# drnatebrown/col-bwt

Measured on AMD Instinct MI355X. Metric: query bases/s, higher is better.
Workload: dtype int64

## Files before the change

### col-bwt_amd/__init__.py

```python
import ctypes as C
import os

import numpy as np

_HERE = os.path.dirname(os.path.abspath(__file__))
LIB_PATH = os.path.join(_HERE, "libcolbwt.so")
HEADER_PATH = os.path.join(os.path.dirname(_HERE), "include", "colbwt.h")

EXPORTS = (
    "colbwt_version", "colbwt_last_error", "colbwt_index_open", "colbwt_index_open_memory",
    "colbwt_index_open_layout", "colbwt_index_open_memory_layout",
    "colbwt_index_open_devices", "colbwt_index_open_memory_devices",
    "colbwt_index_close", "colbwt_index_info", "colbwt_query_batch", "colbwt_query_batch_u32",
    "colbwt_query_device", "colbwt_query_device_ordered", "colbwt_query_file", "colbwt_query_file_binary",
    "colbwt_binary_to_text", "colbwt_synth_index_bytes", "colbwt_synth_index", "colbwt_synth_index_thr", "colbwt_pml_pack_device", "colbwt_read_end_mask_device", "colbwt_pml_unpack_device",
    "colbwt_index_cid_dictionary", "colbwt_cid_code_bits", "colbwt_cid_pack_device", "colbwt_cid_unpack_device",
    "colbwt_synth_reads_device", "colbwt_build_col_pml", "colbwt_build_col_pml_arrays",
    "colbwt_col_split", "colbwt_col_split_arrays", "colbwt_col_split_error",
    "colbwt_rlbwt_build_text", "colbwt_rlbwt_build_files", "colbwt_rlbwt_get", "colbwt_rlbwt_free", "colbwt_rlbwt_error",
    "colbwt_count_batch", "colbwt_count_device", "colbwt_count_file",
    "colbwt_index_attach_locate", "colbwt_index_attach_locate_memory", "colbwt_locate_docs", "colbwt_locate_batch",
    "colbwt_locate_device", "colbwt_locate_file",
    "colbwt_rlbwt_build_text_locate", "colbwt_rlbwt_build_files_locate", "colbwt_rlbwt_write_locate",
)

LOCATE_NONE = (1 << 64) - 1


class ColbwtError(RuntimeError):
    def __init__(self, code, msg):
        super().__init__(f"colbwt error {code}: {msg}")
        self.code = code


class Info(C.Structure):
    _fields_ = [("bwt_r", C.c_uint64), ("n", C.c_uint64), ("r", C.c_uint64), ("sigma", C.c_uint32),
                ("device", C.c_uint32), ("device_bytes", C.c_uint64), ("layout", C.c_uint32),
                ("layout_shape", C.c_uint32), ("table_rows", C.c_uint64), ("n_devices", C.c_uint32),
                ("reserved_", C.c_uint32)]


class Stats(C.Structure):
    _fields_ = [("n_reads", C.c_uint64), ("n_bases", C.c_uint64), ("h2d_ms", C.c_double),
                ("kernel_ms", C.c_double), ("d2h_ms", C.c_double), ("algorithmic_bytes", C.c_uint64)]

    def as_dict(self):
        return {k: getattr(self, k) for k, _ in self._fields_}


_lib = None


def lib():
    global _lib
    if _lib is not None:
        return _lib
    if not os.path.exists(LIB_PATH):
        raise ColbwtError(-100, f"{LIB_PATH} not built: run __graft_entry__.build() "
                                "(the query path has no CPU fallback)")
    try:
        import torch
    except ImportError:
        pass
    L = C.CDLL(LIB_PATH)
    vp, u64, i32 = C.c_void_p, C.c_uint64, C.c_int
    L.colbwt_version.restype = C.c_char_p
    L.colbwt_last_error.restype = C.c_char_p
    L.colbwt_index_open.argtypes = [C.c_char_p, vp, i32, C.POINTER(vp)]
    L.colbwt_index_open_memory.argtypes = [vp, u64, vp, i32, C.POINTER(vp)]
    L.colbwt_index_open_layout.argtypes = [C.c_char_p, vp, i32, i32, C.POINTER(vp)]
    L.colbwt_index_open_memory_layout.argtypes = [vp, u64, vp, i32, i32, C.POINTER(vp)]
    L.colbwt_index_open_devices.argtypes = [C.c_char_p, vp, C.POINTER(i32), i32, i32, C.POINTER(vp)]
# ... 396 lines not shown
```

### col-bwt_amd/csrc/capi.hip

```cpp
#include <fcntl.h>
#include <hip/hip_runtime.h>
#include <stdlib.h>
#include <string.h>
#include <sys/mman.h>
#include <sys/stat.h>
#include <unistd.h>

#include <algorithm>
#include <atomic>
#include <chrono>
#include <condition_variable>
#include <deque>
#include <mutex>
#include <string>
#include <thread>
#include <vector>

#include "../../include/colbwt.h"
#include "bin_writer.h"
#include "count_query.h"
#include "fasta_parallel.h"
#include "fastx_reader.h"
#include "index.h"
#include "locate_query.h"
// ... 797 lines not shown
            const std::string msg = "replica on device " + std::to_string(devices[k]) + ": " + g_err;
            delete first;
            return fail(rc, msg);
        }
        first->more.push_back(rep);
    }
    *out = first;
    return COLBWT_OK;
}

int colbwt_index_open_devices(const char *prefix_or_file, const colbwt_widths *widths, const int *devices, int n_devices,
                              int layout, colbwt_index **out) {
    if (!prefix_or_file || !out) return fail(COLBWT_ERR_ARG, "null argument");
    *out = nullptr;
    MappedFile mf;
    const int rc = map_index_file(prefix_or_file, mf);
    return rc != COLBWT_OK ? rc : colbwt_index_open_memory_devices(mf.data, mf.len, widths, devices, n_devices, layout, out);
}

void colbwt_index_close(colbwt_index *idx) { delete idx; }

int colbwt_index_info(const colbwt_index *idx, colbwt_info *out) {
    if (!idx || !out) return fail(COLBWT_ERR_ARG, "null argument");
    out->bwt_r = idx->ix.bwt_r();
    out->n = idx->ix.n();
    out->r = idx->ix.r();
    out->sigma = idx->ix.sigma();
    out->device = (uint32_t)idx->ix.device();
    out->device_bytes = idx->ix.device_bytes() + idx->loc.bytes();
    out->layout = (uint32_t)idx->ix.layout();
    out->layout_shape = idx->ix.line_rows() ? (idx->ix.table_fat().steps << 8) | kFatSlotSteps : 0;
    out->table_rows = idx->ix.table_rows();
    out->n_devices = 1 + (uint32_t)idx->more.size();
    out->reserved_ = 0;
    return COLBWT_OK;
}

int colbwt_query_batch(colbwt_index *idx, const uint8_t *bases, const uint64_t *read_off, uint64_t n_reads,
                       uint16_t *pml, uint8_t *cid, colbwt_stats *stats) {
    return query_batch_all<uint16_t>(idx, bases, read_off, n_reads, pml, cid, stats);
}

int colbwt_query_batch_u32(colbwt_index *idx, const uint8_t *bases, const uint64_t *read_off, uint64_t n_reads,
                           uint32_t *pml, uint8_t *cid, colbwt_stats *stats) {
    return query_batch_all<uint32_t>(idx, bases, read_off, n_reads, pml, cid, stats);
}

int colbwt_query_device(colbwt_index *idx, const uint8_t *d_bases, const uint64_t *d_read_off, uint64_t n_reads,
                        uint64_t n_bases, void *d_pml, int pml_bytes, uint8_t *d_cid, void *hip_stream,
                        colbwt_stats *stats) {
    return colbwt_query_device_ordered(idx, d_bases, d_read_off, n_reads, n_bases, d_pml, pml_bytes, d_cid, nullptr,
                                       hip_stream, stats);
}

int colbwt_query_device_ordered(colbwt_index *idx, const uint8_t *d_bases, const uint64_t *d_read_off,
                                uint64_t n_reads, uint64_t n_bases, void *d_pml, int pml_bytes, uint8_t *d_cid,
                                const uint32_t *d_order, void *hip_stream, colbwt_stats *stats) {
    auto bad_argument = [&]() -> const char * {
        if (pml_bytes != 2 && pml_bytes != 4) return "pml_bytes must be 2 or 4";
        if (n_reads == 0) return nullptr;
        if (!d_bases || !d_read_off || !d_pml || !d_cid) return "null device pointer";
        if (((uintptr_t)d_bases & 15) || ((uintptr_t)d_pml & 31) || ((uintptr_t)d_cid & 15))
            return "d_bases/d_cid must be 16-byte aligned and d_pml 32-byte aligned";
        return nullptr;
    };
    return device_entry(idx, d_bases, n_reads, n_bases, hip_stream, kAlgBytesPerBase, stats, bad_argument,
                        [&](const Index &ix, hipStream_t stream) {
// ... 405 lines not shown
```

### col-bwt_amd/csrc/fat2_query.hip

```cpp
#include <hip/hip_runtime.h>
#include <stdint.h>

#include "device_layout.h"
#include "fat_cursor.h"
#include "fat_layout.h"
#include "lane_io.h"
#include "lane_out.h"
#include "query_kernels.h"

namespace colbwt {

namespace {

constexpr uint32_t kOffMis0 = 0xFFFFFFFCu;
constexpr uint32_t kOffMis1 = 0xFFFFFFFBu;

#ifdef COLBWT_COUNT_TRIPS
#define FAT2_STAT(k) (++stat[k])
#else
#define FAT2_STAT(k) ((void)0)
#endif

__device__ __forceinline__ uint32_t mis_slot(const uint8_t *top, uint32_t own, uint32_t c) {
    const uint32_t aidx = top[own], cidx = top[c];
    const uint32_t slot = cidx < aidx ? cidx : cidx - 1;
    return cidx < 4 && slot < kFatSlots ? slot : kFatSlots;
}

template <int K, typename PmlT, bool kDeep>
__global__ __launch_bounds__(kQueryBlock)
void fat2_query_kernel(FatTable T, const uint8_t *__restrict__ bases, const uint64_t *__restrict__ read_off,
                       uint64_t n_reads, uint32_t big_reads, uint32_t tail_permille,
                       PmlT *__restrict__ pml, uint8_t *__restrict__ cid) {
    constexpr bool kWide = sizeof(PmlT) == 4;
    __shared__ uint4 s_stage[kWaves][8][64];
    __shared__ uint4 s_win[kWaves][4][64];
    __shared__ uint32_t s_claim;
    __shared__ uint8_t s_top[256];
    const uint32_t wave = threadIdx.x >> 6, lane = threadIdx.x & 63u, g8 = lane & ~7u, p = lane & 7u;
    uint32_t *const s_jx = reinterpret_cast<uint32_t *>(&s_stage[wave][7][48]);
    ChunkPlan plan;
    plan.init(n_reads, big_reads, tail_permille);
    if (threadIdx.x == 0) s_claim = 0;
    s_top[threadIdx.x] = (uint8_t)fat_top_index(T.top4, threadIdx.x);
    __syncthreads();
    uint32_t *const claim = &s_claim;
    ReadCursor rc;
    bool done;
    rc.c_next = threadIdx.x;
    rc.request_chunk(plan, read_off);
    rc.commit();
    done = !rc.enter_chunk(plan, claim);

    OutRuns acc;
    uint32_t trip = 0;
    LaneWindow win;
    win.init(rc.off + rc.k - 1);
    uint4 (*const my_win)[64] = s_win[wave];

    uint32_t j = done ? 0u : T.r - 1;
    uint32_t o = kOffLastPos;
    uint32_t L = 0;
    const uint4 *const my_row = &s_stage[wave][p][g8];

#ifdef COLBWT_COUNT_TRIPS
    unsigned long long stat[8] = {0, 0, 0, 0, 0, 0, 0, 0};
#endif
    while (__any(!done)) {
        bool step_back = false;
        if (!done && rc.k == 0 && !rc.next_in_flight && (rc.r != rc.r_lo || rc.nc_ready)) {
            if (rc.r != rc.r_lo) {
                rc.r -= 1;
                rc.k = rc.off - rc.next_off;
                rc.off = rc.next_off;
                step_back = rc.r > rc.r_lo;
            } else if (kWide || acc.cnt == 0) {
                done = !rc.enter_chunk(plan, claim);
                if (!done) win.init(rc.off + rc.k - 1);
            }
            j = done ? 0u : T.r - 1;
            o = kOffLastPos;
            L = 0;
        }
        const bool live = !done && rc.k != 0;
        uint64_t &k = rc.k;
        const uint64_t g = rc.off + k - 1;

        s_jx[lane] = j;
        wave_sync();
        {
            const uint4 ja = *reinterpret_cast<const uint4 *>(&s_jx[g8]);
            const uint4 jb = *reinterpret_cast<const uint4 *>(&s_jx[g8 + 4]);
            const uint32_t jq[8] = {ja.x, ja.y, ja.z, ja.w, jb.x, jb.y, jb.z, jb.w};
            wave_sync();
#pragma unroll
            for (uint32_t q = 0; q < 8; ++q)
                __builtin_amdgcn_global_load_lds(T.lines + (uint64_t)jq[q] * kFatRowBytes + ((p ^ q) << 4), &s_stage[wave][q][0],
                                                 16, 0, 0);
        }
        if (live && win.avail(g) < (k < 8u ? (uint32_t)k : 8u)) win.request(my_win, bases, g);
        if (step_back) { rc.in_next = read_off[rc.r - 1]; rc.next_in_flight = true; }
        if (!done && rc.fetch_pending) rc.request_chunk(plan, read_off);
        lds_dma_landed();
        rc.commit();

        const uint32_t have = live ? win.avail(g) : 0u;
        uint32_t consumed = 0, l_new = 0, keep = 0xFFFFFFFFu, keep1 = 0xFFFFFFFFu;
        uint64_t ids = 0;
        if (!live || have == 0) FAT2_STAT(5);
        if (live && have != 0) {
            const uint64_t W = win.get8(my_win, lane, g);
            const uint32_t left = k < have ? (uint32_t)k : have;
            if (o == kOffMis0 || o == kOffMis1) {
                FAT2_STAT(2);
                const uint32_t h4 = !kDeep && o == kOffMis1 ? 4u : 0u;
                const uint4 e0 = my_row[(h4 + 0u) ^ p], e1 = my_row[(h4 + 1u) ^ p], e2 = my_row[(h4 + 2u) ^ p],
                            e3 = my_row[(h4 + 3u) ^ p];
                const uint32_t carry = L;
                const uint32_t t1 = (e0.y >> 16) & 0xFFu, d1 = e0.y >> 24, v1 = e3.z & 7u;
                uint32_t oc = 4;
                if (left >= 2) {
                    const uint32_t c2 = (uint32_t)(W >> 48) & 0xFFu;
                    const uint32_t s2 = mis_slot(s_top, t1, c2);
                    if (c2 == t1) oc = 0;
                    else if (s2 < kFatSlots && ((v1 >> s2) & 1u)) oc = 1 + s2;
                }
                if (oc < 4) {
                    const uint32_t J = oc == 0 ? e0.z : oc == 1 ? e0.w : oc == 2 ? e1.x : e1.y;
                    const uint32_t rho = oc == 0 ? e1.z : oc == 1 ? e1.w : oc == 2 ? e2.x : e2.y;
                    const uint32_t pw = oc < 2 ? e2.z : e2.w, P = (oc & 1u) ? pw >> 16 : pw & 0xFFFFu;
                    const uint32_t ch = (e3.x >> (8 * oc)) & 0xFFu, cd = (e3.y >> (8 * oc)) & 0xFFu;
                    const uint32_t vo = (e3.z >> (4 + 4 * oc)) & 7u;
                    consumed = 2;
                    l_new = 1;
                    keep = oc == 0 ? 0xFFFFFFFFu : 0u;
                    ids = (uint64_t)(d1 | (carry << 8));
                    L = oc == 0 ? 1u : 0u;
                    uint32_t nJ = J, nP = P, nrho = rho, nch = ch, ncd = cd, nv = vo, seen = 2;
                    if constexpr (kDeep) {
                        if (left >= 3 && ((uint32_t)(W >> 40) & 0xFFu) == ch) {
                            const uint4 f0 = my_row[4u ^ p], f1 = my_row[5u ^ p], f2 = my_row[6u ^ p], f3 = my_row[7u ^ p];
                            nJ = oc == 0 ? f0.x : oc == 1 ? f0.y : oc == 2 ? f0.z : f0.w;
                            nrho = oc == 0 ? f1.x : oc == 1 ? f1.y : oc == 2 ? f1.z : f1.w;
                            const uint32_t pw2 = oc < 2 ? f2.x : f2.y;
                            nP = (oc & 1u) ? pw2 >> 16 : pw2 & 0xFFFFu;
                            nch = (f2.z >> (8 * oc)) & 0xFFu;
// ... 90 lines not shown
                    } else {
                        consumed = steps - skip;
                        l_new = L + consumed;
                    }
                    L = l_new;
                    ids = steps ? CID >> (8u * (8u - steps)) : 0ull;
                    if (k == consumed) {
                    } else if (to_entry) {
                        FAT2_STAT(6);
                        j = T.slot_line0 + (kDeep ? e_next : e_next >> 1);
                        o = kDeep ? kOffMis0 : kOffMis0 - (e_next & 1u);
                        L = carry;
                    } else if (own_jump) {
                        const uint32_t e = steps - 1;
                        const uint32_t I = reinterpret_cast<const uint32_t *>(&my_row[((kFatI / 16) + (e >> 2)) ^ p])[e & 3u];
                        const uint32_t Oh = reinterpret_cast<const uint16_t *>(&my_row[((kFatO / 16) + (e >> 3)) ^ p])[e & 7u];
                        const uint64_t cuts = (uint64_t)r1.y | ((uint64_t)r1.z << 32);
                        const uint32_t cut = (uint32_t)(cuts >> (8 * e)) & 0xFFu, cut_a = cut & 0xFu, len_b = cut >> 4;
                        j = I;
                        if (cut_a != kSKCutNone && o >= cut_a) {
                            j += 1;
                            o -= cut_a;
                            if (len_b != kSKCutNone && o >= len_b) {
                                j += 1;
                                o -= len_b;
                            }
                        } else {
                            o += Oh;
                        }
                    }
                }
            }
            if constexpr (kWide) {
                for (uint32_t e = 0; e < consumed; ++e) {
                    pml[g - consumed + 1 + e] = (PmlT)((e < 2 ? keep : keep1) ? l_new - e : 0u);
                    cid[g - consumed + 1 + e] = (uint8_t)(ids >> (8 * e));
                }
            } else {
                acc.push_run(consumed, l_new, keep, keep1, (uint32_t)ids, (uint32_t)(ids >> 32));
            }
            k -= consumed;
        }
        wave_sync();
        if constexpr (!kWide) {
#ifdef COLBWT_ABL_NO_FLUSH
            if ((trip & (OutRuns::kPeriod - 1)) == OutRuns::kPeriod - 1) acc.cnt = acc.cnt > 90 ? 1 : 0;
#else
            if ((trip & (OutRuns::kPeriod - 1)) == OutRuns::kPeriod - 1)
                acc.flush_wave((uint16_t *)pml, cid, rc.off + rc.k, !done, rc.k == 0 && rc.r == rc.r_lo, &s_stage[wave][0][0], lane);
#endif
        }
        ++trip;
        wave_sync();
    }
#ifdef COLBWT_COUNT_TRIPS
    for (int q = 0; q < 8; ++q) atomicAdd(&g_fat_stats[q], stat[q]);
#endif
}

template <int K>
void launch_steps2(const FatTable &T, const uint8_t *d_bases, const uint64_t *d_read_off, uint64_t n_reads, uint64_t n_bases,
                   void *d_pml, int pml_bytes, uint8_t *d_cid, hipStream_t stream) {
    const bool deep = T.entry_shift == 7;
    if (pml_bytes == 2 && deep) launch_persistent<fat2_query_kernel<K, uint16_t, true>>(T, d_bases, d_read_off, n_reads, n_bases, (uint16_t *)d_pml, d_cid, stream);
    else if (pml_bytes == 2) launch_persistent<fat2_query_kernel<K, uint16_t, false>>(T, d_bases, d_read_off, n_reads, n_bases, (uint16_t *)d_pml, d_cid, stream);
    else if (deep) launch_persistent<fat2_query_kernel<K, uint32_t, true>>(T, d_bases, d_read_off, n_reads, n_bases, (uint32_t *)d_pml, d_cid, stream);
    else launch_persistent<fat2_query_kernel<K, uint32_t, false>>(T, d_bases, d_read_off, n_reads, n_bases, (uint32_t *)d_pml, d_cid, stream);
}

}

void launch_fat2_query(const FatTable &T, const uint8_t *d_bases, const uint64_t *d_read_off, uint64_t n_reads, uint64_t n_bases,
// ... 21 lines not shown
```

### col-bwt_amd/csrc/fat_build.hip

```cpp
#include <hip/hip_runtime.h>
#include <stdint.h>

#include <functional>
#include <string>
#include <vector>

#include "../../include/colbwt.h"
#include "dev_mem.h"
#include "device_layout.h"
#include "fat_layout.h"
#include "jump_tables.h"
#include "lf_device.h"
#include "query_kernels.h"
#include "read_sampler.h"
#include "refine.h"

namespace colbwt {

namespace {

struct PlainLevel {
    const uint64_t *idx;
    const uint32_t *I;
    const uint16_t *O;
    const uint16_t *meta;
    const uint64_t *thr;
    const uint8_t *org;
    uint64_t n;
    uint32_t r;
};

struct PlainBuffers {
    DevPtr idx, I, O, meta, thr, org;
    void release() {
        for (DevPtr *p : {&idx, &I, &O, &meta, &thr, &org}) p->reset();
    }
};

struct SrcPlain {
    PlainLevel T;
    __device__ __forceinline__ uint32_t cuts(uint32_t, uint64_t (&)[kHintSlots]) const { return 0; }
    __device__ __forceinline__ bool origin_start(uint32_t i, uint64_t b) const { return b == T.idx[i] && T.org[i]; }
// ... 310 lines not shown
    const uint32_t r_new = (uint32_t)total;
    SK_TRY(buf.idx.alloc(((uint64_t)r_new + 2) * sizeof(uint64_t)));
    SK_TRY(buf.I.alloc(((uint64_t)r_new + 1) * sizeof(uint32_t)));
    SK_TRY(buf.O.alloc(((uint64_t)r_new + 1) * sizeof(uint16_t)));
    SK_TRY(buf.meta.alloc(((uint64_t)r_new + 1) * sizeof(uint16_t)));
    SK_TRY(buf.thr.alloc(((uint64_t)r_new + 1) * sizeof(uint64_t)));
    SK_TRY(buf.org.alloc((uint64_t)r_new + 1));
    SK_TRY(park.alloc(((uint64_t)r_new + 1) * sizeof(uint64_t)));
    uint64_t *const d_idx = buf.idx.as<uint64_t>(), *const d_thr = buf.thr.as<uint64_t>(), *const d_park = park.as<uint64_t>();
    uint32_t *const d_I = buf.I.as<uint32_t>(), *const d_first = first.as<uint32_t>();
    uint16_t *const d_O = buf.O.as<uint16_t>(), *const d_meta = buf.meta.as<uint16_t>();
    uint8_t *const d_org = buf.org.as<uint8_t>();
    const uint32_t rblocks = (uint32_t)((src_rows + 255) / 256);
    hipLaunchKernelGGL(plain_emit_kernel<Src>, dim3(rblocks), dim3(256), 0, 0, S, (const uint32_t *)d_first, d_idx, d_I, d_meta,
                       d_thr, d_org, d_park, r_new);
    SK_TRY(hipGetLastError());
    SK_TRY(hipStreamSynchronize(0));
    const uint32_t nblocks = (uint32_t)(((uint64_t)r_new + 255) / 256);
    hipLaunchKernelGGL(plain_link_kernel, dim3(nblocks), dim3(256), 0, 0, (const uint32_t *)d_first, (const uint64_t *)d_idx,
                       (const uint64_t *)d_park, d_I, d_O, r_new);
    SK_TRY(hipGetLastError());
    SK_TRY(hipStreamSynchronize(0));
    out.idx = d_idx;
    out.I = d_I;
    out.O = d_O;
    out.meta = d_meta;
    out.thr = d_thr;
    out.org = d_org;
    out.n = n;
    out.r = r_new;
    return COLBWT_OK;
}

constexpr uint64_t kDeepReserve = 32ull << 30;

template <int K>
int build_fat_steps(const DevTable &T1, const HintChars &chars, int mismatch_lines, FatTable &out, FatBuffers &buf, std::string &err,
                    const std::function<void()> &source_done, int &failed_level) {
    failed_level = 2;
    const uint8_t *cmap = T1.cmap;
    const uint32_t sigma = T1.sigma;
    PlainLevel cur{};
    PlainBuffers cur_buf;
    LoadClock clock;
    {
        const SrcL1 s1{T1, chars};
        const int rc = refine_plain(s1, T1.r, T1.n, cur, cur_buf, err);
        if (rc != COLBWT_OK) return rc;
    }
    clock.lap("  refinement level 2");
    source_done();
    clock.lap("  one-step tables freed");
    for (int level = 3; level <= K; ++level) {
        failed_level = level;
        PlainLevel next{};
        PlainBuffers next_buf;
        const SrcPlain sp{cur};
        const int rc = refine_plain(sp, cur.r, cur.n, next, next_buf, err);
        if (rc != COLBWT_OK) return rc;
        cur_buf.release();
        cur = next;
        cur_buf.idx = std::move(next_buf.idx);
        cur_buf.I = std::move(next_buf.I);
        cur_buf.O = std::move(next_buf.O);
        cur_buf.meta = std::move(next_buf.meta);
        cur_buf.thr = std::move(next_buf.thr);
// ... 51 lines not shown
        const uint8_t *const d_org = cur.org;
        hipLaunchKernelGGL(org_flags_kernel, dim3(nblocks), dim3(256), 0, 0, d_org, r, d_rho);
        SK_TRY(hipGetLastError());
        uint64_t n_rho = 0;
        {
            const int rc = exclusive_scan_u32(d_rho, r, n_rho, err);
            if (rc != COLBWT_OK) return rc;
        }
        if (mismatch_lines == 3) {
            const uint64_t deep_bytes = ((uint64_t)r + 1 + n_rho * kFatSlots) * kFatRowBytes;
            mismatch_lines = deep_bytes + kDeepReserve <= dev_available_bytes() ? 2 : 1;
        }
        const uint32_t entry_shift = mismatch_lines == 2 ? 7u : 6u;
        mis_lines = ((n_rho * kFatSlots << entry_shift) + kFatRowBytes - 1) / kFatRowBytes;
        if ((uint64_t)r + 1 + mis_lines > 0xFFFFFFFEull) {
            err = "line rows + mismatch lines need " + std::to_string((uint64_t)r + 1 + mis_lines) + " lines (> 2^32-2)";
            return COLBWT_ERR_NOMEM;
        }
        out.n_rho = (uint32_t)n_rho;
        out.slot_line0 = r + 1;
        out.entry_shift = entry_shift;
        SK_TRY(rho_first_buf.alloc((n_rho + 1) * sizeof(uint32_t)));
        SK_TRY(sflags_buf.alloc((uint64_t)r + 1));
        d_rho_first = rho_first_buf.as<uint32_t>();
        d_sflags = sflags_buf.as<uint8_t>();
        hipLaunchKernelGGL(rho_kernel, dim3(nblocks), dim3(256), 0, 0, d_org, r, d_rho, d_rho_first);
        SK_TRY(hipGetLastError());
        hipLaunchKernelGGL(fat_slot_flags_kernel, dim3(nblocks), dim3(256), 0, 0, cur, out, (const uint32_t *)d_rho,
                           (const uint32_t *)d_rho_first, d_sflags);
        SK_TRY(hipGetLastError());
        SK_TRY(hipStreamSynchronize(0));
        clock.lap("  origin rows, entry flags");
    }
    {
        PlainAllocScope whole;
        SK_TRY(buf.lines.alloc(((uint64_t)r + 1 + mis_lines) * kFatRowBytes));
    }
    clock.lap("  lines allocated");
    uint8_t *const d_lines = buf.lines.as<uint8_t>();
    SK_TRY(hipMemset(d_lines + (uint64_t)r * kFatRowBytes, 0, kFatRowBytes));
    if (mismatch_lines) {
        hipLaunchKernelGGL((fat_pack_kernel<K, true>), dim3(nblocks), dim3(256), 0, 0, cur, out, (const uint32_t *)d_rho,
                           (const uint8_t *)d_sflags, d_lines);
        SK_TRY(hipGetLastError());
        uint8_t *const d_entries = d_lines + ((uint64_t)r + 1) * kFatRowBytes;
        if (mis_lines) SK_TRY(hipMemset(d_entries + (mis_lines - 1) * kFatRowBytes, 0, kFatRowBytes));
        const uint64_t n_entries = (uint64_t)out.n_rho * kFatSlots;
        if (mismatch_lines == 2)
            hipLaunchKernelGGL(fat_mis_pack_kernel<true>, dim3((uint32_t)((n_entries + 255) / 256)), dim3(256), 0, 0, cur, out,
                               (const uint32_t *)d_rho, (const uint32_t *)d_rho_first, (const uint8_t *)d_sflags, d_entries);
        else
            hipLaunchKernelGGL(fat_mis_pack_kernel<false>, dim3((uint32_t)((n_entries + 255) / 256)), dim3(256), 0, 0, cur, out,
                               (const uint32_t *)d_rho, (const uint32_t *)d_rho_first, (const uint8_t *)d_sflags, d_entries);
    } else {
        hipLaunchKernelGGL((fat_pack_kernel<K, false>), dim3(nblocks), dim3(256), 0, 0, cur, out, (const uint32_t *)nullptr,
                           (const uint8_t *)nullptr, d_lines);
    }
    SK_TRY(hipGetLastError());
    SK_TRY(hipStreamSynchronize(0));
    out.lines = d_lines;
    clock.lap("  lines packed");
    buf.idx = std::move(cur_buf.idx);
    buf.thr = std::move(cur_buf.thr);
    cur_buf.release();
    clock.lap("  level arrays freed");
    return COLBWT_OK;
}

struct FatView {
    FatTable T;
    struct Row {
        uint32_t i1, o1_len, ch;
    };
    __device__ __forceinline__ uint64_t n() const { return T.n; }
    __device__ __forceinline__ uint32_t rows() const { return T.r; }
    __device__ __forceinline__ uint64_t idx(uint32_t j) const { return T.idx[j]; }
    __device__ __forceinline__ Row load(uint32_t j) const {
        const uint32_t *p = reinterpret_cast<const uint32_t *>(T.lines + (uint64_t)j * kFatRowBytes);
        Row w;
        w.i1 = p[kFatI / 4];
        w.o1_len = fat_half(p, kFatO) | (fat_half(p, kFatLen) << 16);
        w.ch = fat_byte(p, kFatCh + 7);
        return w;
    }
    __device__ __forceinline__ uint32_t ch(const Row &w) const { return w.ch; }
    __device__ __forceinline__ uint32_t lf_row(const Row &w) const { return w.i1; }
    __device__ __forceinline__ uint32_t lf_off(const Row &w) const { return w.o1_len & 0xFFFFu; }
    __device__ __forceinline__ uint64_t len(uint32_t, const Row &w) const { return w.o1_len >> 16; }
};

__global__ __launch_bounds__(256) void fat_synth_reads_kernel(FatView V, uint64_t n_reads, uint32_t m, uint32_t sub_permille,
                                                              uint64_t seed, uint8_t *__restrict__ bases,
                                                              uint64_t *__restrict__ read_off) {
    const uint64_t rd = (uint64_t)blockIdx.x * 256 + threadIdx.x;
// ... 45 lines not shown
```

### col-bwt_amd/csrc/fat_layout.h

```cpp
#pragma once
#include <hip/hip_runtime.h>
#include <stdint.h>

#include "device_layout.h"

namespace colbwt {

#define COLBWT_FAT_STEPS(X) X(4) X(5) X(6) X(7) X(8)

constexpr uint32_t kFatRowBytes = 128;
constexpr uint32_t kFatSlots = 3;
constexpr uint32_t kFatSlotSteps = 2;
constexpr uint32_t kFatOwnOther = 7;
constexpr uint32_t kFatCh = 0, kFatCid = 8, kFatLen = 16, kFatFlags = 18, kFatCut = 20, kFatI = 32, kFatO = 64,
                   kFatSlot0 = 80, kFatSlotBytes = 16;
constexpr uint32_t kFatSlotP = 8, kFatSlotCh2 = 12, kFatSlotCid2 = 13;
constexpr uint32_t kFatVal = 28, kFatRho = 80;
constexpr uint32_t kMisBytes = 64, kMisJ1 = 0, kMisP1 = 1, kMisJ = 2, kMisRho = 6, kMisP = 10, kMisCh = 12, kMisCid = 13, kMisVal = 14;
constexpr uint32_t kMisDeep = 16;

struct FatTable {
    const uint8_t *lines;
    const uint8_t *chr;
    const uint64_t *idx;
    const uint64_t *thr;
    const uint32_t *next_tbl;
    const uint32_t *prev_tbl;
    const uint8_t *cmap;
    uint64_t n;
    uint32_t r;
    uint32_t sigma;
    uint32_t nblk;
    uint32_t steps;
    uint32_t top4;
    uint32_t slot_line0;
    uint32_t n_rho;
    uint32_t entry_shift;
};

__device__ __forceinline__ uint32_t fat_byte(const uint32_t *w, uint32_t off) { return (w[off >> 2] >> (8 * (off & 3u))) & 0xFFu; }
__device__ __forceinline__ uint32_t fat_half(const uint32_t *w, uint32_t off) { return (w[off >> 2] >> (8 * (off & 2u))) & 0xFFFFu; }

__device__ __forceinline__ uint32_t fat_top_index(uint32_t top4, uint32_t c) {
    uint32_t x = 4;
    x = ((top4 >> 24) & 0xFFu) == c ? 3u : x;
    x = ((top4 >> 16) & 0xFFu) == c ? 2u : x;
    x = ((top4 >> 8) & 0xFFu) == c ? 1u : x;
    x = (top4 & 0xFFu) == c ? 0u : x;
    return x;
}

__device__ __forceinline__ uint32_t fat_succ_char(const FatTable &T, uint32_t i, uint32_t c, uint32_t cidx) {
    const uint32_t blk = i >> kBlockShift;
    const uint64_t lim = (((uint64_t)blk + 1) << kBlockShift);
    const uint64_t end = lim < T.r ? lim : T.r;
    for (uint64_t s = (uint64_t)i + 1; s < end; ++s)
        if (T.chr[s] == c) return (uint32_t)s;
    if (blk + 1 < T.nblk) return T.next_tbl[(uint64_t)(blk + 1) * T.sigma + cidx];
    return kNone;
}
__device__ __forceinline__ uint32_t fat_pred_char(const FatTable &T, uint32_t i, uint32_t c, uint32_t cidx) {
    const uint32_t blk = i >> kBlockShift;
    const uint32_t first = blk << kBlockShift;
    for (uint32_t q = i; q > first;) {
        --q;
        if (T.chr[q] == c) return q;
    }
    if (blk > 0) return T.prev_tbl[(uint64_t)blk * T.sigma + cidx];
    return kNone;
}
// ... 3 lines not shown
```

### col-bwt_amd/csrc/lane_out.h

```cpp
#pragma once
#include <hip/hip_runtime.h>
#include <stdint.h>

#include "lane_io.h"

#ifdef COLBWT_ABL_NO_STORES
#define COLBWT_ABL_IF if (ltop == 0xFFFFFFF1u)
#else
#define COLBWT_ABL_IF
#endif

namespace colbwt {

struct OutRuns {
    static constexpr uint32_t kBlock = 64;
    static constexpr uint32_t kPeriod = 4;
    static constexpr uint32_t kSlotQ = 6, kItemQ = 4;
    static constexpr uint32_t lds_q(uint32_t slots) { return slots * kSlotQ + 2 * slots * kItemQ; }

    uint32_t z0a = 0, z0b = 0, z0c = 0, z1a = 0, z1b = 0, z1c = 0;
    uint32_t ltop = 0;
    uint32_t c0 = 0, c1 = 0, c2 = 0, c3 = 0, c4 = 0, c5 = 0, c6 = 0, c7 = 0, c8 = 0, c9 = 0, c10 = 0, c11 = 0, c12 = 0, c13 = 0, c14 = 0, c15 = 0, c16 = 0, c17 = 0, c18 = 0, c19 = 0, c20 = 0, c21 = 0, c22 = 0, c23 = 0;
    uint32_t cnt = 0;

    __device__ __forceinline__ void push_run(uint32_t n, uint32_t l_new, uint32_t keep, uint32_t keep1, uint32_t ids_lo,
                                             uint32_t ids_hi) {
        const uint32_t in_run = (1u << n) - 1u;
        uint32_t p0 = l_new < n ? 1u << l_new : 0u;
        p0 |= (keep ? 0u : 3u) & in_run;
        p0 |= (keep1 ? 0u : 0xCu) & in_run;
        const uint32_t top = (1u << n) >> 1;
        const uint32_t p1 = (keep & keep1) != 0u && l_new == n ? top : 0u;
        z0c = (uint32_t)(((((uint64_t)z0c << 32) | z0b) << n) >> 32);
        z0b = (uint32_t)(((((uint64_t)z0b << 32) | z0a) << n) >> 32);
        z0a = (z0a << n) | p0;
        z1c = (uint32_t)(((((uint64_t)z1c << 32) | z1b) << n) >> 32);
        z1b = (uint32_t)(((((uint64_t)z1b << 32) | z1a) << n) >> 32);
        z1a = (z1a << n) | p1;
        const bool d4 = n & 8u, d2 = n & 4u;
        c23 = d4 ? c21 : c23;
        c22 = d4 ? c20 : c22;
        c21 = d4 ? c19 : c21;
        c20 = d4 ? c18 : c20;
        c19 = d4 ? c17 : c19;
        c18 = d4 ? c16 : c18;
        c17 = d4 ? c15 : c17;
        c16 = d4 ? c14 : c16;
        c15 = d4 ? c13 : c15;
        c14 = d4 ? c12 : c14;
        c13 = d4 ? c11 : c13;
        c12 = d4 ? c10 : c12;
        c11 = d4 ? c9 : c11;
        c10 = d4 ? c8 : c10;
        c9 = d4 ? c7 : c9;
        c8 = d4 ? c6 : c8;
        c7 = d4 ? c5 : c7;
        c6 = d4 ? c4 : c6;
        c5 = d4 ? c3 : c5;
        c4 = d4 ? c2 : c4;
        c3 = d4 ? c1 : c3;
        c2 = d4 ? c0 : c2;
        c1 = d4 ? 0u : c1;
        c0 = d4 ? 0u : c0;
        c23 = d2 ? c22 : c23;
        c22 = d2 ? c21 : c22;
// ... 14 lines not shown
        c7 = d2 ? c6 : c7;
        c6 = d2 ? c5 : c6;
        c5 = d2 ? c4 : c5;
        c4 = d2 ? c3 : c4;
        c3 = d2 ? c2 : c3;
        c2 = d2 ? c1 : c2;
        c1 = d2 ? c0 : c1;
        c0 = d2 ? 0u : c0;
        const uint32_t sel8 = 0x07060504u - 0x01010101u * (n & 3u);
        c23 = __builtin_amdgcn_perm(c23, c22, sel8);
        c22 = __builtin_amdgcn_perm(c22, c21, sel8);
        c21 = __builtin_amdgcn_perm(c21, c20, sel8);
        c20 = __builtin_amdgcn_perm(c20, c19, sel8);
        c19 = __builtin_amdgcn_perm(c19, c18, sel8);
        c18 = __builtin_amdgcn_perm(c18, c17, sel8);
        c17 = __builtin_amdgcn_perm(c17, c16, sel8);
        c16 = __builtin_amdgcn_perm(c16, c15, sel8);
        c15 = __builtin_amdgcn_perm(c15, c14, sel8);
        c14 = __builtin_amdgcn_perm(c14, c13, sel8);
        c13 = __builtin_amdgcn_perm(c13, c12, sel8);
        c12 = __builtin_amdgcn_perm(c12, c11, sel8);
        c11 = __builtin_amdgcn_perm(c11, c10, sel8);
        c10 = __builtin_amdgcn_perm(c10, c9, sel8);
        c9 = __builtin_amdgcn_perm(c9, c8, sel8);
        c8 = __builtin_amdgcn_perm(c8, c7, sel8);
        c7 = __builtin_amdgcn_perm(c7, c6, sel8);
        c6 = __builtin_amdgcn_perm(c6, c5, sel8);
        c5 = __builtin_amdgcn_perm(c5, c4, sel8);
        c4 = __builtin_amdgcn_perm(c4, c3, sel8);
        c3 = __builtin_amdgcn_perm(c3, c2, sel8);
        c2 = __builtin_amdgcn_perm(c2, c1, sel8);
        c1 = __builtin_amdgcn_perm(c1, c0, sel8);
        c0 = __builtin_amdgcn_perm(c0, 0u, sel8);
        const uint32_t mlo = n >= 4 ? 0xFFFFFFFFu : (1u << (8 * n)) - 1u;
        const uint32_t mhi = n >= 8 ? 0xFFFFFFFFu : (n > 4 ? (1u << (8 * (n - 4))) - 1u : 0u);
        c0 |= ids_lo & mlo;
        c1 |= ids_hi & mhi;
        cnt += n;
    }

    static __device__ __forceinline__ void shr96(uint64_t &lo, uint32_t &hi, uint32_t s) {
        if (s >= 64) {
            lo = (uint64_t)(hi >> (s - 64));
            hi = 0;
        } else if (s) {
            lo = (lo >> s) | ((uint64_t)hi << (64 - s));
            hi = s < 32 ? hi >> s : 0u;
        }
    }
    static __device__ __forceinline__ uint64_t low64_from(uint32_t a, uint32_t b, uint32_t c, uint32_t s) {
        uint64_t lo = ((uint64_t)b << 32) | a;
        uint32_t hi = c;
        shr96(lo, hi, s);
        return lo;
    }
    __device__ __forceinline__ uint32_t park_item(uint4 *item, uint32_t slot, uint32_t e_lo, uint32_t count, uint64_t addr, uint32_t lt) const {
        const uint32_t o_lo = (uint32_t)addr & (kBlock - 1), o_hi = o_lo + count;
        const uint64_t in_item = count >= 64 ? ~0ull : (1ull << count) - 1ull;
        const uint64_t Z0 = (low64_from(z0a, z0b, z0c, e_lo) & in_item) << o_lo;
        const uint64_t Z1 = (low64_from(z1a, z1b, z1c, e_lo) & in_item) << o_lo;
        const uint32_t z0w[2] = {(uint32_t)Z0, (uint32_t)(Z0 >> 32)}, z1w[2] = {(uint32_t)Z1, (uint32_t)(Z1 >> 32)};
        uint32_t pm[8];
        uint32_t v = lt;
#pragma unroll
        for (int p = 7; p >= 0; --p) {
            const uint32_t b0 = (z0w[p >> 2] >> (8 * (p & 3))) & 0xFFu, b1 = (z1w[p >> 2] >> (8 * (p & 3))) & 0xFFu;
            pm[p] = (v & 0xFFFFu) | (b0 << 16) | (b1 << 24);
            const uint32_t lo_p = o_lo > 8u * p ? o_lo : 8u * p, hi_p = o_hi < 8u * p + 8u ? o_hi : 8u * p + 8u;
            if (hi_p > lo_p) {
                const uint32_t bits = b0 | b1;
                if (bits) {
// ... 144 lines not shown
```

### include/colbwt.h

```cpp
#ifndef COLBWT_H
#define COLBWT_H

#include <stddef.h>
#include <stdint.h>

#ifdef __cplusplus
extern "C" {
#endif

#define COLBWT_OK 0
#define COLBWT_ERR_ARG (-1)
#define COLBWT_ERR_IO (-2)
#define COLBWT_ERR_FORMAT (-3)
#define COLBWT_ERR_NO_DEVICE (-4)
#define COLBWT_ERR_HIP (-5)
#define COLBWT_ERR_NOMEM (-6)

typedef struct colbwt_index colbwt_index;

typedef struct colbwt_widths {
    uint32_t bwt_bytes;
    uint32_t run_bytes;
    uint32_t len_bytes;
    uint32_t id_bits;
} colbwt_widths;

typedef struct colbwt_info {
    uint64_t bwt_r;
    uint64_t n;
    uint64_t r;
    uint32_t sigma;
    uint32_t device;
    uint64_t device_bytes;
    uint32_t layout;
    uint32_t layout_shape;
    uint64_t table_rows;
    uint32_t n_devices;
    uint32_t reserved_;
} colbwt_info;

typedef struct colbwt_stats {
    uint64_t n_reads;
    uint64_t n_bases;
    double h2d_ms;
    double kernel_ms;
    double d2h_ms;
    uint64_t algorithmic_bytes;
} colbwt_stats;

const char *colbwt_version(void);
const char *colbwt_last_error(void);

int colbwt_index_open(const char *prefix_or_file, const colbwt_widths *widths, int device,
                      colbwt_index **out);
int colbwt_index_open_memory(const void *col_pml_bytes, uint64_t len, const colbwt_widths *widths,
                             int device, colbwt_index **out);
#define COLBWT_LAYOUT_AUTO 0
#define COLBWT_LAYOUT_ONE_STEP 1
#define COLBWT_LAYOUT_TWO_STEP 2
#define COLBWT_LAYOUT_THREE_STEP 3
#define COLBWT_LAYOUT_LINE_ROWS 4
#define COLBWT_LAYOUT_LINE_ROWS_STEPS(K) (COLBWT_LAYOUT_LINE_ROWS | ((K) << 8))
#define COLBWT_LAYOUT_MISMATCH_LINES 5
#define COLBWT_LAYOUT_MISMATCH_LINES_STEPS(K) (COLBWT_LAYOUT_MISMATCH_LINES | ((K) << 8))
#define COLBWT_LAYOUT_MISMATCH_LINES_DEEP 6
#define COLBWT_LAYOUT_MISMATCH_LINES_DEEP_STEPS(K) (COLBWT_LAYOUT_MISMATCH_LINES_DEEP | ((K) << 8))
int colbwt_index_open_layout(const char *prefix_or_file, const colbwt_widths *widths, int device, int layout,
                             colbwt_index **out);
int colbwt_index_open_memory_layout(const void *col_pml_bytes, uint64_t len, const colbwt_widths *widths,
                                    int device, int layout, colbwt_index **out);
int colbwt_index_open_devices(const char *prefix_or_file, const colbwt_widths *widths, const int *devices,
// ... 119 lines not shown
```

Baseline: 141.7 billion.

## Add precomputed start k-mer table to skip initial backward steps per read

Builds a table indexed by the last k bases of each read (up to 14) that stores the fat-table state, match lengths, mismatch mask and colour ids after k backward steps from the start. The query kernel looks up this entry on entering a read and consumes k bases at once, instead of performing k individual row traversals. The output accumulator gains a generic push that takes precomputed masks and up to 16 id bytes. The cost is extra device memory, a build-time level-by-level kernel, more window loading and some extra per-iteration branching in the hot loop.

```diff
diff --git a/col-bwt_amd/__init__.py b/col-bwt_amd/__init__.py
--- a/col-bwt_amd/__init__.py
+++ b/col-bwt_amd/__init__.py
@@ -37,7 +37,7 @@
     _fields_ = [("bwt_r", C.c_uint64), ("n", C.c_uint64), ("r", C.c_uint64), ("sigma", C.c_uint32),
                 ("device", C.c_uint32), ("device_bytes", C.c_uint64), ("layout", C.c_uint32),
                 ("layout_shape", C.c_uint32), ("table_rows", C.c_uint64), ("n_devices", C.c_uint32),
-                ("reserved_", C.c_uint32)]
+                ("start_kmer", C.c_uint32)]
 
 
 class Stats(C.Structure):
diff --git a/col-bwt_amd/csrc/capi.hip b/col-bwt_amd/csrc/capi.hip
--- a/col-bwt_amd/csrc/capi.hip
+++ b/col-bwt_amd/csrc/capi.hip
@@ -853,7 +853,7 @@
     out->layout_shape = idx->ix.line_rows() ? (idx->ix.table_fat().steps << 8) | kFatSlotSteps : 0;
     out->table_rows = idx->ix.table_rows();
     out->n_devices = 1 + (uint32_t)idx->more.size();
-    out->reserved_ = 0;
+    out->start_kmer = idx->ix.line_rows() ? idx->ix.table_fat().start_k : 0;
     return COLBWT_OK;
 }
 
diff --git a/col-bwt_amd/csrc/fat2_query.hip b/col-bwt_amd/csrc/fat2_query.hip
--- a/col-bwt_amd/csrc/fat2_query.hip
+++ b/col-bwt_amd/csrc/fat2_query.hip
@@ -14,6 +14,7 @@
 
 constexpr uint32_t kOffMis0 = 0xFFFFFFFCu;
 constexpr uint32_t kOffMis1 = 0xFFFFFFFBu;
+constexpr uint32_t kOffStart0 = 0xFFFFFFF4u;
 
 #ifdef COLBWT_COUNT_TRIPS
 #define FAT2_STAT(k) (++stat[k])
@@ -61,6 +62,8 @@
     uint32_t j = done ? 0u : T.r - 1;
     uint32_t o = kOffLastPos;
     uint32_t L = 0;
+    const uint32_t kS = T.start_k;
+    bool want_key = !done && kS != 0 && rc.k > kS;
     const uint4 *const my_row = &s_stage[wave][p][g8];
 
 #ifdef COLBWT_COUNT_TRIPS
@@ -81,10 +84,29 @@
             j = done ? 0u : T.r - 1;
             o = kOffLastPos;
             L = 0;
+            want_key = !done && kS != 0 && rc.k > kS;
         }
         const bool live = !done && rc.k != 0;
         uint64_t &k = rc.k;
         const uint64_t g = rc.off + k - 1;
+        if (want_key && win.avail(g) >= kS) {
+            const uint32_t after = OutRuns::kPeriod - 1u - (trip & (OutRuns::kPeriod - 1u));
+            const uint64_t W0 = win.get8(my_win, lane, g), W1 = win.get8(my_win, lane, g - 8u);
+            uint32_t key = 0, bad = 0;
+#pragma unroll
+            for (uint32_t i = 0; i < kStartMaxK; ++i) {
+                if (i < kS) {
+                    const uint32_t d = s_top[(uint32_t)((i < 8u ? W0 >> (8u * (7u - i)) : W1 >> (8u * (15u - i)))) & 0xFFu];
+                    bad |= d;
+                    key = (key << 2) | (d & 3u);
+                }
+            }
+            want_key = false;
+            if (bad < 4u && (kWide || acc.cnt + kS + (uint32_t)K * after <= OutRuns::kCapacity)) {
+                j = T.start_line0 + (key >> 2);
+                o = kOffStart0 + (key & 3u);
+            }
+        }
 
         s_jx[lane] = j;
         wave_sync();
@@ -98,7 +120,11 @@
                 __builtin_amdgcn_global_load_lds(T.lines + (uint64_t)jq[q] * kFatRowBytes + ((p ^ q) << 4), &s_stage[wave][q][0],
                                                  16, 0, 0);
         }
-        if (live && win.avail(g) < (k < 8u ? (uint32_t)k : 8u)) win.request(my_win, bases, g);
+        {
+            uint32_t need = want_key ? kS : (k < 8u ? (uint32_t)k : 8u);
+            if (kS != 0 && rc.r != rc.r_lo && k + kS <= 48u) need = (uint32_t)k + kS;
+            if (live && win.avail(g) < need) win.request(my_win, bases, g);
+        }
         if (step_back) { rc.in_next = read_off[rc.r - 1]; rc.next_in_flight = true; }
         if (!done && rc.fetch_pending) rc.request_chunk(plan, read_off);
         lds_dma_landed();
@@ -107,11 +133,31 @@
         const uint32_t have = live ? win.avail(g) : 0u;
         uint32_t consumed = 0, l_new = 0, keep = 0xFFFFFFFFu, keep1 = 0xFFFFFFFFu;
         uint64_t ids = 0;
+        uint32_t ids2 = 0, ids3 = 0, z0s = 0, z1s = 0;
+        bool from_start = false;
         if (!live || have == 0) FAT2_STAT(5);
         if (live && have != 0) {
             const uint64_t W = win.get8(my_win, lane, g);
             const uint32_t left = k < have ? (uint32_t)k : have;
-            if (o == kOffMis0 || o == kOffMis1) {
+            if (want_key) {
+#ifdef COLBWT_COUNT_TRIPS
+                stat[7] += 1ull << 32;
+#endif
+            } else if (o - kOffStart0 < 4u) {
+                FAT2_STAT(7);
+                const uint32_t h = 2u * (o - kOffStart0);
+                const uint4 e0 = my_row[h ^ p], e1 = my_row[(h + 1u) ^ p];
+                consumed = kS;
+                from_start = true;
+                z0s = e0.z;
+                z1s = (e0.z >> (kS - 1u)) & 1u ? 0u : 1u << (kS - 1u);
+                ids = (uint64_t)e0.w | ((uint64_t)e1.x << 32);
+                ids2 = e1.y;
+                ids3 = e1.z;
+                j = e0.x;
+                o = e0.y & 0xFFFFu;
+                L = e0.y >> 16;
+            } else if (o == kOffMis0 || o == kOffMis1) {
                 FAT2_STAT(2);
                 const uint32_t h4 = !kDeep && o == kOffMis1 ? 4u : 0u;
                 const uint4 e0 = my_row[(h4 + 0u) ^ p], e1 = my_row[(h4 + 1u) ^ p], e2 = my_row[(h4 + 2u) ^ p],
@@ -268,12 +314,25 @@
                 }
             }
             if constexpr (kWide) {
-                for (uint32_t e = 0; e < consumed; ++e) {
-                    pml[g - consumed + 1 + e] = (PmlT)((e < 2 ? keep : keep1) ? l_new - e : 0u);
-                    cid[g - consumed + 1 + e] = (uint8_t)(ids >> (8 * e));
+                if (from_start) {
+                    uint32_t v = 0;
+                    for (uint32_t i = 0; i < consumed; ++i) {
+                        const uint32_t e = consumed - 1u - i;
+                        v = (z0s >> e) & 1u ? 0u : v + 1u;
+                        const uint32_t w = e < 8u ? (uint32_t)(ids >> (8 * e)) : (e < 12u ? ids2 : ids3) >> (8 * (e & 3u));
+                        pml[g - i] = (PmlT)v;
+                        cid[g - i] = (uint8_t)w;
+                    }
+                } else {
+                    for (uint32_t e = 0; e < consumed; ++e) {
+                        pml[g - consumed + 1 + e] = (PmlT)((e < 2 ? keep : keep1) ? l_new - e : 0u);
+                        cid[g - consumed + 1 + e] = (uint8_t)(ids >> (8 * e));
+                    }
                 }
             } else {
-                acc.push_run(consumed, l_new, keep, keep1, (uint32_t)ids, (uint32_t)(ids >> 32));
+                uint32_t m0 = z0s, m1 = z1s;
+                if (!from_start) OutRuns::run_masks(consumed, l_new, keep, keep1, m0, m1);
+                acc.push(consumed, m0, m1, (uint32_t)ids, (uint32_t)(ids >> 32), ids2, ids3);
             }
             k -= consumed;
         }
diff --git a/col-bwt_amd/csrc/fat_build.hip b/col-bwt_amd/csrc/fat_build.hip
--- a/col-bwt_amd/csrc/fat_build.hip
+++ b/col-bwt_amd/csrc/fat_build.hip
@@ -8,6 +8,7 @@
 #include "../../include/colbwt.h"
 #include "dev_mem.h"
 #include "device_layout.h"
+#include "fat_cursor.h"
 #include "fat_layout.h"
 #include "jump_tables.h"
 #include "lf_device.h"
@@ -384,6 +385,81 @@
     return COLBWT_OK;
 }
 
+__device__ __forceinline__ bool start_step(const FatTable &T, uint32_t &j, uint32_t &o, uint32_t c, uint32_t &id) {
+    const uint8_t *row = T.lines + (uint64_t)j * kFatRowBytes;
+    id = row[kFatCid + 7];
+    const bool match = row[kFatCh + 7] == c;
+    if (!match) {
+        const uint32_t cidx = T.cmap[c];
+        uint32_t nj = j, no = o;
+        if (cidx != kAbsent && fat_threshold_scan(T, nj, no, c, cidx)) {
+            row = T.lines + (uint64_t)nj * kFatRowBytes;
+            const uint32_t len = row[kFatLen] | (uint32_t)row[kFatLen + 1] << 8;
+            j = nj;
+            o = no == kOffPred ? len - 1 : 0u;
+        }
+    }
+    const uint32_t I = *reinterpret_cast<const uint32_t *>(row + kFatI);
+    const uint32_t Oh = row[kFatO] | (uint32_t)row[kFatO + 1] << 8;
+    const uint32_t cut = row[kFatCut], cut_a = cut & 0xFu, len_b = cut >> 4;
+    j = I;
+    if (cut_a != kSKCutNone && o >= cut_a) {
+        j += 1;
+        o -= cut_a;
+        if (len_b != kSKCutNone && o >= len_b) {
+            j += 1;
+            o -= len_b;
+        }
+    } else {
+        o += Oh;
+    }
+    for (;;) {
+        row = T.lines + (uint64_t)j * kFatRowBytes;
+        const uint32_t len = row[kFatLen] | (uint32_t)row[kFatLen + 1] << 8;
+        if (o < len) break;
+        if (j + 1 >= T.r) {
+            o = len - 1;
+            break;
+        }
+        o -= len;
+        j += 1;
+    }
+    return match;
+}
+
+__global__ __launch_bounds__(256) void start_level_kernel(FatTable T, uint32_t level, uint8_t *__restrict__ table) {
+    const uint64_t P = (uint64_t)blockIdx.x * 256 + threadIdx.x;
+    if (P >> (2 * level)) return;
+    const uint32_t sh = 2 * (T.start_k - level);
+    uint4 *const at = reinterpret_cast<uint4 *>(table + ((P << sh) * kStartBytes));
+    uint32_t j, o, L, mis;
+    uint4 ids;
+    if (level == 0) {
+        j = T.r - 1;
+        const uint8_t *row = T.lines + (uint64_t)j * kFatRowBytes;
+        o = (row[kFatLen] | (uint32_t)row[kFatLen + 1] << 8) - 1u;
+        L = 0;
+        mis = 0;
+        ids = make_uint4(0, 0, 0, 0);
+    } else {
+        const uint4 a = at[0], b = at[1];
+        j = a.x;
+        o = a.y & 0xFFFFu;
+        L = a.y >> 16;
+        mis = a.z;
+        ids = make_uint4(a.w, b.x, b.y, b.z);
+    }
+    const uint4 up = make_uint4(ids.x << 8, (ids.y << 8) | (ids.x >> 24), (ids.z << 8) | (ids.y >> 24), (ids.w << 8) | (ids.z >> 24));
+    for (uint32_t c = 0; c < 4; ++c) {
+        uint32_t nj = j, no = o, id = 0;
+        const bool match = start_step(T, nj, no, (T.top4 >> (8 * c)) & 0xFFu, id);
+        const uint32_t nL = match ? L + 1u : 0u;
+        uint4 *const dst = reinterpret_cast<uint4 *>(table + (((P << 2) + c) << (sh - 2)) * kStartBytes);
+        dst[0] = make_uint4(nj, no | nL << 16, (mis << 1) | (match ? 0u : 1u), up.x | id);
+        dst[1] = make_uint4(up.y, up.z, up.w, 0u);
+    }
+}
+
 constexpr uint64_t kDeepReserve = 32ull << 30;
 
 template <int K>
@@ -501,9 +577,39 @@
         SK_TRY(hipStreamSynchronize(0));
         clock.lap("  origin rows, entry flags");
     }
+    uint64_t start_lines = 0;
+    if (mismatch_lines) {
+        const uint64_t base_bytes = ((uint64_t)r + 1 + mis_lines) * kFatRowBytes;
+        const uint64_t resident = base_bytes + (uint64_t)r * 17;
+        uint32_t k = 0;
+        const char *e = getenv("COLBWT_START_KMER");
+        if (e && *e) {
+            const long v = strtol(e, nullptr, 10);
+            if (v < 0 || v > (long)kStartMaxK) {
+                err = "COLBWT_START_KMER must be 0 .. " + std::to_string(kStartMaxK);
+                return COLBWT_ERR_ARG;
+            }
+            k = (uint32_t)v;
+        } else {
+            const uint64_t avail = dev_available_bytes();
+            for (uint32_t t = kStartMaxK; t >= 1 && k == 0; --t) {
+                const uint64_t bytes = (1ull << (2 * t)) * kStartBytes;
+                if (bytes * 16 <= resident && base_bytes + bytes + kDeepReserve <= avail) k = t;
+            }
+        }
+        if (k) {
+            start_lines = ((1ull << (2 * k)) * kStartBytes + kFatRowBytes - 1) / kFatRowBytes;
+            if ((uint64_t)r + 1 + mis_lines + start_lines > 0xFFFFFFFEull) {
+                err = "line rows + mismatch lines + start table need more than 2^32-2 lines";
+                return COLBWT_ERR_NOMEM;
+            }
+            out.start_k = k;
+            out.start_line0 = (uint32_t)((uint64_t)r + 1 + mis_lines);
+        }
+    }
     {
         PlainAllocScope whole;
-        SK_TRY(buf.lines.alloc(((uint64_t)r + 1 + mis_lines) * kFatRowBytes));
+        SK_TRY(buf.lines.alloc(((uint64_t)r + 1 + mis_lines + start_lines) * kFatRowBytes));
     }
     clock.lap("  lines allocated");
     uint8_t *const d_lines = buf.lines.as<uint8_t>();
@@ -529,6 +635,18 @@
     SK_TRY(hipStreamSynchronize(0));
     out.lines = d_lines;
     clock.lap("  lines packed");
+    if (out.start_k) {
+        uint8_t *const d_start = d_lines + (uint64_t)out.start_line0 * kFatRowBytes;
+        if (start_lines * kFatRowBytes > ((uint64_t)kStartBytes << (2 * out.start_k)))
+            SK_TRY(hipMemset(d_start, 0, start_lines * kFatRowBytes));
+        for (uint32_t level = 0; level < out.start_k; ++level) {
+            const uint64_t parents = 1ull << (2 * level);
+            hipLaunchKernelGGL(start_level_kernel, dim3((uint32_t)((parents + 255) / 256)), dim3(256), 0, 0, out, level, d_start);
+            SK_TRY(hipGetLastError());
+        }
+        SK_TRY(hipStreamSynchronize(0));
+        clock.lap("  start table");
+    }
     buf.idx = std::move(cur_buf.idx);
     buf.thr = std::move(cur_buf.thr);
     cur_buf.release();
diff --git a/col-bwt_amd/csrc/fat_layout.h b/col-bwt_amd/csrc/fat_layout.h
--- a/col-bwt_amd/csrc/fat_layout.h
+++ b/col-bwt_amd/csrc/fat_layout.h
@@ -18,6 +18,7 @@
 constexpr uint32_t kFatVal = 28, kFatRho = 80;
 constexpr uint32_t kMisBytes = 64, kMisJ1 = 0, kMisP1 = 1, kMisJ = 2, kMisRho = 6, kMisP = 10, kMisCh = 12, kMisCid = 13, kMisVal = 14;
 constexpr uint32_t kMisDeep = 16;
+constexpr uint32_t kStartBytes = 32, kStartMaxK = 14;
 
 struct FatTable {
     const uint8_t *lines;
@@ -36,6 +37,8 @@
     uint32_t slot_line0;
     uint32_t n_rho;
     uint32_t entry_shift;
+    uint32_t start_line0;
+    uint32_t start_k;
 };
 
 __device__ __forceinline__ uint32_t fat_byte(const uint32_t *w, uint32_t off) { return (w[off >> 2] >> (8 * (off & 3u))) & 0xFFu; }
diff --git a/col-bwt_amd/csrc/lane_out.h b/col-bwt_amd/csrc/lane_out.h
--- a/col-bwt_amd/csrc/lane_out.h
+++ b/col-bwt_amd/csrc/lane_out.h
@@ -15,6 +15,7 @@
 struct OutRuns {
     static constexpr uint32_t kBlock = 64;
     static constexpr uint32_t kPeriod = 4;
+    static constexpr uint32_t kCapacity = 96;
     static constexpr uint32_t kSlotQ = 6, kItemQ = 4;
     static constexpr uint32_t lds_q(uint32_t slots) { return slots * kSlotQ + 2 * slots * kItemQ; }
 
@@ -23,14 +24,17 @@
     uint32_t c0 = 0, c1 = 0, c2 = 0, c3 = 0, c4 = 0, c5 = 0, c6 = 0, c7 = 0, c8 = 0, c9 = 0, c10 = 0, c11 = 0, c12 = 0, c13 = 0, c14 = 0, c15 = 0, c16 = 0, c17 = 0, c18 = 0, c19 = 0, c20 = 0, c21 = 0, c22 = 0, c23 = 0;
     uint32_t cnt = 0;
 
-    __device__ __forceinline__ void push_run(uint32_t n, uint32_t l_new, uint32_t keep, uint32_t keep1, uint32_t ids_lo,
-                                             uint32_t ids_hi) {
+    static __device__ __forceinline__ void run_masks(uint32_t n, uint32_t l_new, uint32_t keep, uint32_t keep1, uint32_t &p0,
+                                                     uint32_t &p1) {
         const uint32_t in_run = (1u << n) - 1u;
-        uint32_t p0 = l_new < n ? 1u << l_new : 0u;
+        p0 = l_new < n ? 1u << l_new : 0u;
         p0 |= (keep ? 0u : 3u) & in_run;
         p0 |= (keep1 ? 0u : 0xCu) & in_run;
         const uint32_t top = (1u << n) >> 1;
-        const uint32_t p1 = (keep & keep1) != 0u && l_new == n ? top : 0u;
+        p1 = (keep & keep1) != 0u && l_new == n ? top : 0u;
+    }
+    __device__ __forceinline__ void push(uint32_t n, uint32_t p0, uint32_t p1, uint32_t ids0, uint32_t ids1, uint32_t ids2,
+                                         uint32_t ids3) {
         z0c = (uint32_t)(((((uint64_t)z0c << 32) | z0b) << n) >> 32);
         z0b = (uint32_t)(((((uint64_t)z0b << 32) | z0a) << n) >> 32);
         z0a = (z0a << n) | p0;
@@ -111,11 +115,20 @@
         c2 = __builtin_amdgcn_perm(c2, c1, sel8);
         c1 = __builtin_amdgcn_perm(c1, c0, sel8);
         c0 = __builtin_amdgcn_perm(c0, 0u, sel8);
-        const uint32_t mlo = n >= 4 ? 0xFFFFFFFFu : (1u << (8 * n)) - 1u;
-        const uint32_t mhi = n >= 8 ? 0xFFFFFFFFu : (n > 4 ? (1u << (8 * (n - 4))) - 1u : 0u);
-        c0 |= ids_lo & mlo;
-        c1 |= ids_hi & mhi;
+        c0 |= ids0 & bytes_mask(n);
+        c1 |= ids1 & bytes_mask(n - 4u);
+        c2 |= ids2 & bytes_mask(n - 8u);
+        c3 |= ids3 & bytes_mask(n - 12u);
         cnt += n;
+    }
+    static __device__ __forceinline__ uint32_t bytes_mask(uint32_t m) {
+        return (int32_t)m >= 4 ? 0xFFFFFFFFu : ((int32_t)m <= 0 ? 0u : (1u << (8 * m)) - 1u);
+    }
+    __device__ __forceinline__ void push_run(uint32_t n, uint32_t l_new, uint32_t keep, uint32_t keep1, uint32_t ids_lo,
+                                             uint32_t ids_hi) {
+        uint32_t p0, p1;
+        run_masks(n, l_new, keep, keep1, p0, p1);
+        push(n, p0, p1, ids_lo, ids_hi, 0u, 0u);
     }
 
     static __device__ __forceinline__ void shr96(uint64_t &lo, uint32_t &hi, uint32_t s) {
diff --git a/include/colbwt.h b/include/colbwt.h
--- a/include/colbwt.h
+++ b/include/colbwt.h
@@ -36,7 +36,7 @@
     uint32_t layout_shape;
     uint64_t table_rows;
     uint32_t n_devices;
-    uint32_t reserved_;
+    uint32_t start_kmer;
 } colbwt_info;
 
 typedef struct colbwt_stats {
```

Result: slower. 140.1 billion, median of 2 (-1.1%).
